# WGLab/NanoMod

Measured on AMD Instinct MI355X. Metric: genomic positions/sec (KS + Stouffer), higher is better.
Workload: dtype f32 keys / f64 p-values; 1 GPU; BASELINE.json configs[1]: E. coli 4.6 Mb: 4600000 positions in total (4600000 per GPU), 200 v 200 reads/position, KS + weighted Stouffer window=5; preset=ecoli, positions_total=4600000, positions_per_gpu=4600000, n0=200, n1=200, layout=fixed stride, ties=few, spread_milli=0, outlier_permille=0, rccl_ranks=0, ks_d=float form, bit for bit, parallelism=one GPU, no collective

## Files before the change

### nanomod_amd/csrc/ks_rank.hpp

```cpp
#pragma once
#include <hip/hip_runtime.h>
#include <stdint.h>
#include <type_traits>
#include "rank_stats_packed.hpp"
#include "packed_sort_i16.hpp"
#include "item_claim.hpp"

namespace nmod {

static __device__ const float kKsBig4[4] = {3.4028234663852886e38f, 3.4028234663852886e38f, 3.4028234663852886e38f, 3.4028234663852886e38f};
static __device__ const unsigned kKsInf4[4] = {0x7f800000u, 0x7f800000u, 0x7f800000u, 0x7f800000u};
static __device__ const unsigned kKsPad16[4] = {0x7fff7fffu, 0x7fff7fffu, 0x7fff7fffu, 0x7fff7fffu};

__host__ __device__ constexpr bool ks_packed_sort(int R, int LG, int DTYPE) { return DTYPE == 1 && R == 16 && (LG == 8 || LG == 16); }

template <int R, int LG>
struct KsLayout {
  static constexpr int C = R * LG;
  static constexpr int ROW = LG + 1;
  static constexpr int REGION = R * ROW;
  static constexpr int LAST = (R - 1) * ROW + LG - 1;
  static constexpr int END = LG;
  __device__ static __forceinline__ int word(int i) { return __mul24(i & (R - 1), ROW) + i / R; }
};

__host__ __device__ constexpr int ks_rank_pos_words(int R, int LG) {
  int w = 2 * R * (LG + 1);
  if (LG <= 16) while ((w & 31) != LG) ++w;
  return w;
}

template <typename T>
__device__ __forceinline__ T ks_global_load(const void* p) {
  typedef const T __attribute__((address_space(1)))* GlobalPtr;
  return *(GlobalPtr)(p);
}

typedef float KsF4v __attribute__((ext_vector_type(4)));
typedef short KsS4v __attribute__((ext_vector_type(4)));
typedef KsF4v KsF4 __attribute__((aligned(4)));
typedef KsS4v KsS4 __attribute__((aligned(2)));

template <int R, int LG, int DTYPE>
struct KsRows {
  using T = typename std::conditional<DTYPE == 0, float, int16_t>::type;
  using V4 = typename std::conditional<DTYPE == 0, KsF4, KsS4>::type;
  static constexpr int NK = R / 4;
  V4 v[NK];
  T s[3];

  __device__ __forceinline__ void request(const void* sig, int64_t off, int n, int gl) {
    const T* row = reinterpret_cast<const T*>(sig) + off;
    const T* dummy = ks_packed_sort(R, LG, DTYPE) ? reinterpret_cast<const T*>(kKsPad16) : reinterpret_cast<const T*>(kKsInf4);
    const bool long_row = n >= 4;
#pragma unroll
    for (int k = 0; k < NK; ++k) {
      const int idx = k * (4 * LG) + 4 * gl;
      const int t = n - idx;
      const T* p = (long_row && t > 0) ? row + ((t >= 4) ? idx : n - 4) : dummy;
      v[k] = ks_global_load<V4>(p);
    }
    s[0] = s[1] = s[2] = T(0);
    if (__ballot(!long_row && n > 0) != 0ull) {
#pragma unroll
      for (int e = 0; e < 3; ++e)
        if (!long_row && gl == 0 && e < n) s[e] = ks_global_load<T>(row + e);
    }
  }

  struct Plan { unsigned boff[NK]; int last; bool last_live; };
  __device__ static __forceinline__ Plan plan(int n, int gl) {
    Plan pl;
    pl.last = (n >= 4) ? (n - 1) / (4 * LG) : -1;
    pl.last_live = n >= 4 && n - (pl.last * (4 * LG) + 4 * gl) > 0;
#pragma unroll
    for (int k = 0; k < NK; ++k) {
      const int idx = k * (4 * LG) + 4 * gl;
      const int t = n - idx;
      pl.boff[k] = (n >= 4 && t > 0) ? (unsigned)((t >= 4) ? idx : n - 4) * (unsigned)sizeof(T) : 0u;
    }
    return pl;
  }
  __device__ __forceinline__ void request_uniform(const void* sig, int64_t off, int n, int gl, const Plan& pl) {
    const char* row = reinterpret_cast<const char*>(reinterpret_cast<const T*>(sig) + off);
    const char* dummy = ks_packed_sort(R, LG, DTYPE) ? reinterpret_cast<const char*>(kKsPad16) : reinterpret_cast<const char*>(kKsInf4);
    int last = pl.last;
    asm volatile("" : "+s"(last));
#pragma unroll
    for (int k = 0; k < NK; ++k) {
      const bool live = k < last || (k == last && pl.last_live);
      v[k] = ks_global_load<V4>(live ? row + pl.boff[k] : dummy);
    }
    s[0] = s[1] = s[2] = T(0);
    asm volatile("" : "+v"(gl), "+s"(n));
    if (n < 4) {
#pragma unroll
      for (int e = 0; e < 3; ++e)
        if (gl == 0 && e < n) s[e] = ks_global_load<T>(reinterpret_cast<const T*>(row) + e);
    }
  }

  template <bool UNI = false>
  __device__ __forceinline__ void finish(float (&x)[R], int n, int gl) const {
    const float inf = __builtin_inff();
    if constexpr (UNI) asm volatile("" : "+v"(gl), "+s"(n));
    const bool long_row = n >= 4;
    const bool row_end = long_row && (n & 3) != 0;
#pragma unroll
    for (int k = 0; k < NK; ++k) {
      const int idx = k * (4 * LG) + 4 * gl;
      const int t = long_row ? n - idx : 0;
      if constexpr (DTYPE == 0) {
        x[4 * k + 0] = v[k].x; x[4 * k + 1] = v[k].y; x[4 * k + 2] = v[k].z; x[4 * k + 3] = v[k].w;
        if (UNI ? row_end : (__ballot(t > 0 && t < 4) != 0ull)) {
          x[4 * k + 0] = (t >= 4 || t <= 0) ? x[4 * k + 0] : inf;
          x[4 * k + 1] = (t >= 3 || t <= 0) ? x[4 * k + 1] : inf;
          x[4 * k + 2] = (t >= 2 || t <= 0) ? x[4 * k + 2] : inf;
        }
      } else {
        x[4 * k + 0] = (t >= 4) ? (float)v[k].x : inf;
        x[4 * k + 1] = (t >= 3) ? (float)v[k].y : inf;
        x[4 * k + 2] = (t >= 2) ? (float)v[k].z : inf;
        x[4 * k + 3] = (t >= 1) ? (float)v[k].w : inf;
      }
    }
    if (UNI ? !long_row : (__ballot(!long_row && n > 0) != 0ull)) {
#pragma unroll
      for (int e = 0; e < 3; ++e) x[e] = (!long_row && gl == 0 && e < n) ? (float)s[e] : x[e];
    }
  }

  template <bool UNI = false>
  __device__ __forceinline__ void finish_packed(unsigned (&p)[8], int n, int gl) const {
    static_assert(R == 16, "packed rows: 16 keys per lane");
    if constexpr (UNI) asm volatile("" : "+v"(gl), "+s"(n));
    const bool long_row = n >= 4;
    const bool row_end = long_row && (n & 3) != 0;
#pragma unroll
    for (int k = 0; k < NK; ++k) {
      p[2 * k] = ((unsigned)(unsigned short)v[k].y << 16) | (unsigned)(unsigned short)v[k].x;
      p[2 * k + 1] = ((unsigned)(unsigned short)v[k].w << 16) | (unsigned)(unsigned short)v[k].z;
      const int idx = k * (4 * LG) + 4 * gl;
      const int t = long_row ? n - idx : 0;
      if (UNI ? row_end : (__ballot(t > 0 && t < 4) != 0ull)) {
        if (t == 3) p[2 * k] = (p[2 * k] & 0xffff0000u) | 0x7fffu;
        if (t == 2 || t == 1) p[2 * k] = 0x7fff7fffu;
        if (t == 1) p[2 * k + 1] = (p[2 * k + 1] & 0xffff0000u) | 0x7fffu;
      }
    }
    if (UNI ? !long_row : (__ballot(!long_row && n > 0) != 0ull)) {
      if (!long_row && gl == 0) {
        const unsigned s0 = (0 < n) ? (unsigned)(unsigned short)s[0] : 0x7fffu;
        const unsigned s1 = (1 < n) ? (unsigned)(unsigned short)s[1] : 0x7fffu;
        const unsigned s2 = (2 < n) ? (unsigned)(unsigned short)s[2] : 0x7fffu;
        p[0] = (s1 << 16) | s0;
        p[1] = (0x7fffu << 16) | s2;
      }
    }
  }
};

template <int LG>
__device__ __forceinline__ unsigned seg_allmax_u32(unsigned v) {
  v = max(v, (unsigned)dpp_i<NMOD_QP(1, 0, 3, 2), 0xf, 0xf, true>(0, (int)v));
  v = max(v, (unsigned)dpp_i<NMOD_QP(2, 3, 0, 1), 0xf, 0xf, true>(0, (int)v));
  v = max(v, (unsigned)dpp_i<kDppRowHalfMirror, 0xf, 0xf, true>(0, (int)v));
  if constexpr (LG >= 16) v = max(v, (unsigned)dpp_i<kDppRowMirror, 0xf, 0xf, true>(0, (int)v));
  if constexpr (LG >= 32) v = max(v, (unsigned)__builtin_amdgcn_ds_swizzle((int)v, 0x401F));
  if constexpr (LG == 64) v = max(__builtin_amdgcn_readlane(v, 0), __builtin_amdgcn_readlane(v, 32));
  return v;
}

template <int LG>
__device__ __forceinline__ unsigned seg_exscan_add_u32(unsigned v, int gl) {
  unsigned inc = v;
  auto step = [&](auto tag, int dist) {
    constexpr int C = decltype(tag)::value;
    unsigned t = (unsigned)dpp_i<C, 0xf, 0xf, true>(0, (int)inc);
    inc += (gl >= dist) ? t : 0u;
  };
  step(std::integral_constant<int, kDppRowShr + 1>{}, 1);
  step(std::integral_constant<int, kDppRowShr + 2>{}, 2);
  step(std::integral_constant<int, kDppRowShr + 4>{}, 4);
  if constexpr (LG >= 16) step(std::integral_constant<int, kDppRowShr + 8>{}, 8);
  if constexpr (LG >= 32) {
    unsigned t = (unsigned)dpp_i<kDppRowBcast15, 0xA>(0, (int)inc);
    inc += ((gl & 16) != 0) ? t : 0u;
  }
  if constexpr (LG == 64) {
    unsigned t = (unsigned)dpp_i<kDppRowBcast31, 0xC>(0, (int)inc);
    inc += (gl >= 32) ? t : 0u;
  }
  return inc - v;
}

template <int R, int LG>
__device__ __forceinline__ void seg_sort_any(float (&x)[R], const LaneSel& sel, int lane) {
  seg_sort<R, (LG == 64 ? 32 : LG)>(x, sel, lane);
  if constexpr (LG == 64) merge_lanes<R, 64>(x, sel, lane);
}

template <int R, int LG, bool LE, bool FULL = true>
__device__ __forceinline__ const float* ks_search(const float* base, float x) {
  using Lay = KsLayout<R, LG>;
  const float* p = base;
  bool all = false;
  if constexpr (FULL) {
    const float last = base[Lay::LAST];
    all = LE ? (last <= x) : (last < x);
  }
#pragma unroll
  for (int hc = LG / 2; hc >= 1; hc >>= 1) {
    const float t = p[(R - 1) * Lay::ROW + hc - 1];
    const bool right = LE ? (t <= x) : (t < x);
    p = right ? p + hc : p;
  }
#pragma unroll
  for (int h = R / 2; h >= 1; h >>= 1) {
    const float t = p[(h - 1) * Lay::ROW];
    const bool right = LE ? (t <= x) : (t < x);
    p = right ? p + h * Lay::ROW : p;
  }
  return all ? base + Lay::END : p;
}

struct KsTops { float hi, lo0, lo1, last; };
template <int R, int LG>
__device__ __forceinline__ KsTops ks_tops(const float* base) {
  using Lay = KsLayout<R, LG>;
  auto uni = [](float v) { return __int_as_float(__builtin_amdgcn_readfirstlane(__float_as_int(v))); };
  KsTops t;
  t.hi = uni(base[(R - 1) * Lay::ROW + LG / 2 - 1]);
  t.lo0 = uni(base[(R - 1) * Lay::ROW + LG / 4 - 1]);
  t.lo1 = uni(base[(R - 1) * Lay::ROW + LG / 2 + LG / 4 - 1]);
  t.last = uni(base[Lay::LAST]);
  return t;
}
template <int R, int LG>
__device__ __forceinline__ const float* ks_search_tops(const float* base, float x, const KsTops& t) {
  using Lay = KsLayout<R, LG>;
  static_assert(LG >= 4, "two row levels");
  const bool all = t.last < x;
  const bool r1 = t.hi < x;
  const float t2 = r1 ? t.lo1 : t.lo0;
  const bool r2 = t2 < x;
  const float* p = base + (r1 ? LG / 2 : 0) + (r2 ? LG / 4 : 0);
#pragma unroll
  for (int hc = LG / 8; hc >= 1; hc >>= 1) {
    const float v = p[(R - 1) * Lay::ROW + hc - 1];
    p = (v < x) ? p + hc : p;
  }
#pragma unroll
  for (int h = R / 2; h >= 1; h >>= 1) {
    const float v = p[(h - 1) * Lay::ROW];
    p = (v < x) ? p + h * Lay::ROW : p;
  }
  return all ? base + Lay::END : p;
}

__device__ __forceinline__ double fmax_numbers(double a, double b) {
  double r;
  asm("v_max_f64 %0, %1, %2" : "=v"(r) : "v"(a), "v"(b));
  return r;
}

template <int LG>
__device__ __forceinline__ double seg_allmax_f64(double v) {
  v = fmax_numbers(v, dpp_f64_row(v, 0)); v = fmax_numbers(v, dpp_f64_row(v, 1)); v = fmax_numbers(v, dpp_f64_row(v, 2));
  if constexpr (LG >= 16) v = fmax_numbers(v, dpp_f64_row(v, 3));
  if constexpr (LG >= 32) v = fmax(v, xor16_f64(v));
  if constexpr (LG == 64) v = wave_max_f64(v);
  return v;
}

__device__ __forceinline__ double hist_exact_quot(int c, double n, double r) {
  const double dc = (double)c;
  const double q0 = __dmul_rn(dc, r);
  const double rem = __fma_rn(-q0, n, dc);
  return __fma_rn(rem, r, q0);
}

template <int LG>
__device__ __forceinline__ void seg_moments_packed16(const unsigned (&p)[8], int n, int gl, double& mean, double& m2, double rcp_n = 0.0) {
  int s1 = 0;
  double s2 = 0.0;
#pragma unroll
  for (int j = 0; j < 8; ++j) {
    const int lo = (int)(short)(p[j] & 0xffffu), hi = (int)p[j] >> 16;
    s1 += lo + hi;
    const double dl = (double)lo, dh = (double)hi;
    s2 = __fma_rn(dl, dl, s2);
    s2 = __fma_rn(dh, dh, s2);
  }
  int valid = 0;
#pragma unroll
  for (int k = 0; k < 4; ++k) valid += min(max(n - (k * 4 * LG + 4 * gl), 0), 4);
  valid = (n >= 4) ? valid : ((gl == 0) ? n : 0);
  const int npad = 16 - valid;
  s1 -= 32767 * npad;
  s2 -= 1073676289.0 * (double)npad;
  unsigned v = (unsigned)s1;
  v += (unsigned)dpp_i<NMOD_QP(1, 0, 3, 2), 0xf, 0xf, true>(0, (int)v);
  v += (unsigned)dpp_i<NMOD_QP(2, 3, 0, 1), 0xf, 0xf, true>(0, (int)v);
  v += (unsigned)dpp_i<kDppRowHalfMirror, 0xf, 0xf, true>(0, (int)v);
  if constexpr (LG >= 16) v += (unsigned)dpp_i<kDppRowMirror, 0xf, 0xf, true>(0, (int)v);
  const double S1 = (double)(int)v;
  const double S2 = seg_allsum_f64<LG>(s2);
  const double dn = (double)n;
  const double rn = (rcp_n != 0.0) ? rcp_n : 1.0 / dn;
  milli_moments(0.0, S1, S2, dn, rn, mean, m2);
}

template <int R, int LG, int DTYPE, bool FLAGS = false, bool UNIFORM = false>
__global__ __launch_bounds__(64 * kWavesPerBlock, (R <= 16 ? 4 : 2))
void ks_rank_kernel(RankStatsArgs args) {
  static_assert(!(UNIFORM && FLAGS), "the float64 front end keeps the generic instance");
  static_assert(LG == 8 || LG == 16 || LG == 32 || LG == 64, "lanes per sorted group");
  static_assert(R >= 8 && R <= 32 && (R & (R - 1)) == 0, "registers per lane");
  constexpr int PW = 64 / LG;
  using Lay = KsLayout<R, LG>;
  constexpr int ROW = Lay::ROW;
  constexpr int POS_WORDS = ks_rank_pos_words(R, LG);
  constexpr int HIST_OFF = Lay::REGION;
  extern __shared__ __attribute__((aligned(16))) float lds_all[];

  const int lane = threadIdx.x & 63;
  const int wave = __builtin_amdgcn_readfirstlane(threadIdx.x >> 6);
  const int gl = lane & (LG - 1);
  const int slot = lane / LG;
  float* keys = lds_all + (wave * PW + slot) * POS_WORDS;
  unsigned* hist = reinterpret_cast<unsigned*>(keys + HIST_OFF);
  const int e0 = gl * R;

  const float inf = __builtin_inff();
  LaneSel sel;
#pragma unroll
  for (int b = 0; b < 6; ++b) sel.s[b] = ((lane >> b) & 1) ? inf : -inf;
  for (int r = gl; r < R; r += LG) keys[r * ROW + Lay::END] = inf;
  const bool uniform = args.stride0 > 0 && args.stride1 > 0;
  double* recip = reinterpret_cast<double*>(lds_all + kWavesPerBlock * PW * POS_WORDS);
  if (uniform && threadIdx.x == 0) {
    const int64_t a0 = args.stride0 < args.stride1 ? args.stride0 : args.stride1;
    const int64_t a1 = args.stride0 < args.stride1 ? args.stride1 : args.stride0;
    recip[0] = 1.0 / (double)a0; recip[1] = 1.0 / (double)a1;
  }
  __syncthreads();

  int64_t count = args.npos;
  const int32_t* list = nullptr;
  if constexpr (UNIFORM) {
    if (count <= 0) return;
  } else
  if (args.alt_gates != nullptr && args.alt_gates[args.class_id] != 0) {
    count = args.alt_meta[args.class_id];
    list = args.alt_list + args.alt_meta[kClassStride + args.class_id];
  } else if (args.pos_list) {
    count = args.class_meta[args.class_id];
    list = args.pos_list + args.class_meta[kClassStride + args.class_id];
  }
  const int64_t items = (count + PW - 1) / PW;
  const int64_t wave_global = (int64_t)blockIdx.x * kWavesPerBlock + wave;
  const int64_t wave_stride = (int64_t)gridDim.x * kWavesPerBlock;

  struct Item { bool valid, swap; int m, q; int64_t pos, off_s, off_q; };
  const uint32_t items32 = (uint32_t)items;
  const bool u_swap = args.stride1 < args.stride0;
  const int u_m = (int)(u_swap ? args.stride1 : args.stride0), u_q = (int)(u_swap ? args.stride0 : args.stride1);
  const void* const u_sig_s = u_swap ? args.sig1 : args.sig0;
  const void* const u_sig_q = u_swap ? args.sig0 : args.sig1;
  auto describe = [&](uint32_t it) {
    Item d;
    const uint32_t li = min(it, items32) * PW + slot;
    d.valid = li < (uint32_t)count;
    if constexpr (UNIFORM) {
      d.pos = d.valid ? (int64_t)li : 0;
      d.swap = u_swap; d.m = u_m; d.q = u_q;
      d.off_s = (int64_t)((uint64_t)(uint32_t)d.pos * (uint64_t)(uint32_t)u_m);
      d.off_q = (int64_t)((uint64_t)(uint32_t)d.pos * (uint64_t)(uint32_t)u_q);
      return d;
    }
    d.pos = d.valid ? (list ? (int64_t)list[li] : (int64_t)li) : 0;
    int64_t o0 = 0, o1 = 0; int n0 = 0, n1 = 0;
    if (d.valid) {
      if (args.stride0 > 0) { o0 = (int64_t)((uint64_t)(uint32_t)d.pos * (uint64_t)(uint32_t)args.stride0); n0 = (int)args.stride0; }
      else { o0 = args.off0[d.pos]; n0 = (int)(args.off0[d.pos + 1] - o0); }
      if (args.stride1 > 0) { o1 = (int64_t)((uint64_t)(uint32_t)d.pos * (uint64_t)(uint32_t)args.stride1); n1 = (int)args.stride1; }
      else { o1 = args.off1[d.pos]; n1 = (int)(args.off1[d.pos + 1] - o1); }
    }
    d.swap = n1 < n0;
    d.m = d.swap ? n1 : n0; d.q = d.swap ? n0 : n1;
    d.off_s = d.swap ? o1 : o0; d.off_q = d.swap ? o0 : o1;
    return d;
  };
  const float big = 3.4028234663852886e38f;
  using Q4Raw = typename std::conditional<DTYPE == 0, KsF4, KsS4>::type;
  using Q1Raw = typename std::conditional<DTYPE == 0, float, int16_t>::type;
  auto load_q4 = [&](const void* sig, int64_t off, int idx, bool have) -> Q4Raw {
    using T = Q1Raw;
    const T* src = have ? reinterpret_cast<const T*>(sig) + off + idx : reinterpret_cast<const T*>(kKsBig4);
    return ks_global_load<Q4Raw>(src);
  };
  auto q4_values = [&](float (&xq)[4], const Q4Raw& t, bool have) {
    if constexpr (DTYPE == 0) {
      (void)have;
      xq[0] = t.x; xq[1] = t.y; xq[2] = t.z; xq[3] = t.w;
    } else {
      xq[0] = have ? (float)t.x : big; xq[1] = have ? (float)t.y : big;
      xq[2] = have ? (float)t.z : big; xq[3] = have ? (float)t.w : big;
    }
  };
  auto load_q1 = [&](const void* sig, int64_t off, int idx, bool have) -> Q1Raw {
    using T = Q1Raw;
    return ks_global_load<T>(have ? reinterpret_cast<const T*>(sig) + off + idx : reinterpret_cast<const T*>(kKsBig4));
  };
  auto q1_value = [&](Q1Raw v, bool have) -> float {
    if constexpr (DTYPE == 0) { (void)have; return v; }
    else return have ? (float)v : big;
  };

  ItemWalk walk;
  const uint32_t it_first = walk.begin(item_claim_plan<uint32_t>((uint32_t)items, (uint32_t)wave_stride, args.strided_items != 0),
                                      (uint32_t)wave_global, (uint32_t)wave_stride, args.claim + args.class_id, lane);
  Item cur = describe(it_first);
  constexpr bool PACKED = ks_packed_sort(R, LG, DTYPE);
  float x[R];
  unsigned pk[8];
  [[maybe_unused]] typename KsRows<R, LG, DTYPE>::Plan row_plan;
  if constexpr (UNIFORM) row_plan = KsRows<R, LG, DTYPE>::plan(u_m, gl);
  [[maybe_unused]] double u_dm = 0.0, u_dq = 0.0, u_rm = 0.0, u_rq = 0.0;
  if constexpr (UNIFORM) {
    auto uni64 = [](double v) {
      const unsigned long long b = (unsigned long long)__double_as_longlong(v);
      unsigned lo, hi;
      asm("v_readfirstlane_b32 %0, %1" : "=s"(lo) : "v"((unsigned)b));
      asm("v_readfirstlane_b32 %0, %1" : "=s"(hi) : "v"((unsigned)(b >> 32)));
      return __longlong_as_double((long long)(((unsigned long long)hi << 32) | lo));
    };
    u_dm = uni64((double)u_m); u_dq = uni64((double)u_q); u_rm = uni64(recip[0]); u_rq = uni64(recip[1]);
  }
  {
    KsRows<R, LG, DTYPE> first;
    if constexpr (UNIFORM) first.request_uniform(u_sig_s, cur.off_s, u_m, gl, row_plan);
    else first.request(cur.swap ? args.sig1 : args.sig0, cur.off_s, cur.m, gl);
    if constexpr (PACKED) first.template finish_packed<UNIFORM>(pk, cur.m, gl);
    else first.template finish<UNIFORM>(x, cur.m, gl);
  }
  __builtin_amdgcn_s_waitcnt(0x0F70);
  walk.collect();

  for (uint32_t it = it_first, it_next; it < items32; it = it_next) {
    const bool valid = cur.valid;
    const int64_t pos = cur.pos;
    const int m = UNIFORM ? u_m : cur.m, q = UNIFORM ? u_q : cur.q;
    const void* sig_q = UNIFORM ? u_sig_q : (cur.swap ? args.sig0 : args.sig1);
    const int64_t off_q = cur.off_q;

    const int full = q / (4 * LG);
    const int tail = (q - full * (4 * LG) + LG - 1) / LG;
    int full_w = full, tail_w = tail;
    if constexpr (UNIFORM) {
    } else if constexpr (PW > 1) {
      full_w = 0; tail_w = 0;
#pragma unroll
      for (int s = 0; s < PW; ++s) {
        full_w = max(full_w, __builtin_amdgcn_readlane(full, s * LG));
        tail_w = max(tail_w, __builtin_amdgcn_readlane(tail, s * LG));
      }
    } else {
      full_w = __builtin_amdgcn_readfirstlane(full);
      tail_w = __builtin_amdgcn_readfirstlane(tail);
    }
    int slots = (full_w * 4 + tail_w) * LG;
    bool coop = false;
    if constexpr (UNIFORM) {
    } else if constexpr (PW > 1) {
      int coop_cost = 0;
#pragma unroll
      for (int sl = 0; sl < PW; ++sl) {
        const int qs = __builtin_amdgcn_readlane(q, sl * LG);
        const int fs = qs / 256;
        coop_cost += fs * 4 + (qs - fs * 256 + 63) / 64;
      }
      coop = coop_cost < full_w * 4 + tail_w;
    }
    it_next = walk.next(it, lane);
    const Item nxt = describe(it_next);
    KsRows<R, LG, DTYPE> rows_next;
    if constexpr (UNIFORM) rows_next.request_uniform(u_sig_s, nxt.off_s, u_m, gl, row_plan);
    else rows_next.request(nxt.swap ? args.sig1 : args.sig0, nxt.off_s, nxt.m, gl);
    constexpr bool PIPE_COOP = LG == 8;
    auto row_of_slot = [&](int sl, const void*& sg, int64_t& of, int& qn) {
      const int src = sl * LG;
      auto rl64 = [&](unsigned long long v) {
        const unsigned lo = (unsigned)__builtin_amdgcn_readlane((int)(unsigned)v, src);
        const unsigned hi = (unsigned)__builtin_amdgcn_readlane((int)(unsigned)(v >> 32), src);
        return ((unsigned long long)hi << 32) | (unsigned long long)lo;
      };
      sg = reinterpret_cast<const void*>((uintptr_t)rl64((unsigned long long)(uintptr_t)sig_q));
      of = (int64_t)rl64((unsigned long long)off_q);
      qn = __builtin_amdgcn_readlane(q, src);
    };
    const void* sig_c = sig_q; int64_t off_c = off_q; int q_c = q;
    int idx_a = 4 * gl, idx_t = full * (4 * LG) + gl;
    bool have_a = !coop && 0 < full, have_t = !coop && idx_t < q;
    if constexpr (PIPE_COOP) {
      if (coop) {
        row_of_slot(0, sig_c, off_c, q_c);
        idx_a = 4 * lane; idx_t = (q_c / 256) * 256 + lane; have_a = q_c >= 256; have_t = idx_t < q_c;
      }
    }
    Q4Raw ra = load_q4(sig_c, off_c, idx_a, have_a);
    Q1Raw rt = load_q1(sig_c, off_c, idx_t, have_t);

    if constexpr (PACKED) {
      seg_sort_packed16<LG>(pk, lane);
      unpack_sorted16<LG>(pk, x);
    } else {
      seg_sort_any<R, LG>(x, sel, lane);
    }
#pragma unroll
    for (int r = 0; r < R; ++r) keys[r * ROW + gl] = x[r];
    if constexpr (PACKED) {
      int real = m - e0;
      if constexpr (UNIFORM) asm volatile("" : "+v"(real));
#pragma unroll
      for (int r = 0; r < R; ++r)
        if (r >= real) keys[r * ROW + gl] = inf;
    }
#pragma unroll
    for (int r = 0; r < R; ++r) hist[r * ROW + gl] = 0u;
    if (gl == LG - 1) hist[Lay::END] = 0u;
    __builtin_amdgcn_fence(__ATOMIC_RELEASE, "wavefront");
    __builtin_amdgcn_wave_barrier();

    int m_full = m;
    if constexpr (UNIFORM) asm volatile("" : "+s"(m_full));
    const bool s_full = UNIFORM ? (m_full == Lay::C) : (__ballot(m == Lay::C) != 0ull);

    auto rank_and_count = [&](auto nv_tag, auto full_tag, const float* kbase, const float* xq) {
      constexpr int NV = decltype(nv_tag)::value;
      constexpr bool FULL = decltype(full_tag)::value;
      const float* lp[NV];
#pragma unroll
      for (int e = 0; e < NV; ++e) lp[e] = ks_search<R, LG, false, FULL>(kbase, xq[e]);
      unsigned inc[NV];
#pragma unroll
      for (int e = 0; e < NV; ++e) inc[e] = (*lp[e] == xq[e]) ? 0x10001u : 0x10000u;
#pragma unroll
      for (int e = 0; e < NV; ++e) atomicAdd(reinterpret_cast<unsigned*>(const_cast<float*>(lp[e])) + HIST_OFF, inc[e]);
    };

    [[maybe_unused]] auto rank_and_count_tops = [&](auto nv_tag, const float* kbase, const KsTops& tops, const float* xq) {
      constexpr int NV = decltype(nv_tag)::value;
      const float* lp[NV];
#pragma unroll
      for (int e = 0; e < NV; ++e) lp[e] = ks_search_tops<R, LG>(kbase, xq[e], tops);
      unsigned inc[NV];
#pragma unroll
      for (int e = 0; e < NV; ++e) inc[e] = (*lp[e] == xq[e]) ? 0x10001u : 0x10000u;
#pragma unroll
      for (int e = 0; e < NV; ++e) atomicAdd(reinterpret_cast<unsigned*>(const_cast<float*>(lp[e])) + HIST_OFF, inc[e]);
    };

    __builtin_amdgcn_s_waitcnt(0x0F70);
    walk.collect();
    if (!coop) {
#pragma unroll 1
      for (int c = 0; c < full_w; ++c) {
        const Q4Raw rb = UNIFORM ? load_q4(sig_q, off_q, min(c + 1, full - 1) * (4 * LG) + 4 * gl, true)
                                 : load_q4(sig_q, off_q, (c + 1) * (4 * LG) + 4 * gl, c + 1 < full);
        float xa[4];
        q4_values(xa, ra, c < full);
        if (s_full) rank_and_count(std::integral_constant<int, 4>{}, std::true_type{}, keys, xa);
        else rank_and_count(std::integral_constant<int, 4>{}, std::false_type{}, keys, xa);
        ra = rb;
      }
#pragma unroll 1
      for (int c = 0; c < tail_w; ++c) {
        float xq[1] = {q1_value(rt, full * (4 * LG) + c * LG + gl < q)};
        const int idx = full * (4 * LG) + (c + 1) * LG + gl;
        rt = load_q1(sig_q, off_q, idx, idx < q);
        if (s_full) rank_and_count(std::integral_constant<int, 1>{}, std::true_type{}, keys, xq);
        else rank_and_count(std::integral_constant<int, 1>{}, std::false_type{}, keys, xq);
      }
    } else {
      const int cfull = q / 256;
      slots = (cfull * 4 + (q - cfull * 256 + 63) / 64) * 64;
      if constexpr (PIPE_COOP) {
#pragma unroll 1
      for (int sl = 0; sl < PW; ++sl) {
        const void* sig_n = sig_c; int64_t off_n = off_c; int q_n = 0;
        if (sl + 1 < PW) row_of_slot(sl + 1, sig_n, off_n, q_n);
        const int nfs = q_n / 256;
        const Q4Raw na = load_q4(sig_n, off_n, 4 * lane, nfs > 0);
        const Q1Raw nt = load_q1(sig_n, off_n, nfs * 256 + lane, nfs * 256 + lane < q_n);
        const float* kb = lds_all + (wave * PW + sl) * POS_WORDS;
        const int fs = q_c / 256, ts = (q_c - fs * 256 + 63) / 64;
        const KsTops tops = ks_tops<R, LG>(kb);
#pragma unroll 2
        for (int c = 0; c < fs; ++c) {
          const Q4Raw rb = load_q4(sig_c, off_c, min(c + 1, fs - 1) * 256 + 4 * lane, true);
          float xq[4];
          q4_values(xq, ra, true);
          rank_and_count_tops(std::integral_constant<int, 4>{}, kb, tops, xq);
          ra = rb;
        }
#pragma unroll 1
        for (int c = 0; c < ts; ++c) {
          const int idx_now = fs * 256 + c * 64 + lane;
          const Q1Raw r1 = load_q1(sig_c, off_c, idx_now + 64, idx_now + 64 < q_c);
          float xq[1] = {q1_value(rt, idx_now < q_c)};
          rank_and_count_tops(std::integral_constant<int, 1>{}, kb, tops, xq);
          rt = r1;
        }
        sig_c = sig_n; off_c = off_n; q_c = q_n; ra = na; rt = nt;
      }
      } else {
#pragma unroll 1
      for (int sl = 0; sl < PW; ++sl) {
        const int src = sl * LG;
        const int qs = __builtin_amdgcn_readlane(q, src);
        const unsigned long long sp = (unsigned long long)(uintptr_t)sig_q;
        auto rl64 = [&](unsigned long long v) {
          const unsigned lo = (unsigned)__builtin_amdgcn_readlane((int)(unsigned)v, src);
          const unsigned hi = (unsigned)__builtin_amdgcn_readlane((int)(unsigned)(v >> 32), src);
          return ((unsigned long long)hi << 32) | (unsigned long long)lo;
        };
        const void* sigs = reinterpret_cast<const void*>((uintptr_t)rl64(sp));
        const int64_t offs = (int64_t)rl64((unsigned long long)off_q);
        const float* kb = lds_all + (wave * PW + sl) * POS_WORDS;
        const int fs = qs / 256, ts = (qs - fs * 256 + 63) / 64;
#pragma unroll 1
        for (int c = 0; c < fs; ++c) {
          const int idx = c * 256 + 4 * lane;
          float xq[4];
          q4_values(xq, load_q4(sigs, offs, idx, true), true);
          rank_and_count(std::integral_constant<int, 4>{}, std::true_type{}, kb, xq);
        }
#pragma unroll 1
        for (int c = 0; c < ts; ++c) {
          const int idx = fs * 256 + c * 64 + lane;
          float xq[1] = {q1_value(load_q1(sigs, offs, idx, idx < qs), idx < qs)};
          rank_and_count(std::integral_constant<int, 1>{}, std::true_type{}, kb, xq);
        }
      }
      }
    }
    __builtin_amdgcn_fence(__ATOMIC_RELEASE, "wavefront");
    __builtin_amdgcn_wave_barrier();
    if (gl == 0) { const unsigned extra = (unsigned)(slots - q); hist[Lay::word(m)] -= extra << 16; }
    __builtin_amdgcn_fence(__ATOMIC_RELEASE, "wavefront");
    __builtin_amdgcn_wave_barrier();

    unsigned h[R];
#pragma unroll
    for (int r = 0; r < R - 1; ++r) h[r] = hist[(r + 1) * ROW + gl];
    h[R - 1] = hist[gl + 1];
    const unsigned h0 = hist[0];
    unsigned tot = 0;
#pragma unroll
    for (int r = 0; r < R; ++r) tot += h[r];
    const unsigned cum = seg_exscan_add_u32<LG>(tot, gl) + h0;
    unsigned best = 0;
    float s_own[R];
#pragma unroll
    for (int r = 0; r < R; ++r) s_own[r] = keys[r * ROW + gl];
    const float s_next = keys[gl + 1];
    const bool tie_lane = ((tot | h0) & 0xffffu) != 0u;
    bool slow = __ballot(tie_lane) != 0ull;
    if (!slow) {
      float gap = inf;
#pragma unroll
      for (int r = 0; r < R; ++r) gap = fminf(gap, ((r == R - 1) ? s_next : s_own[r + 1]) - s_own[r]);
      slow = __ballot(gap == 0.0f) != 0ull;
    }
    if (!slow) {
      int m_ev = m;
      if constexpr (UNIFORM) asm volatile("" : "+s"(m_ev));
      const int kq_max = __mul24(m_ev - 1, q);
      int kq = min(__mul24(e0, q), kq_max);
      if constexpr (UNIFORM) asm volatile("" : "+v"(kq));
      const int cmax = q - (int)(hist[Lay::word(m)] >> 16);
      int c = min((int)(cum >> 16), cmax);
      int a = __mul24(c, m) - kq;
      int hi = (gl == 0) ? a : -(1 << 30), lo = 1 << 30;
      if (gl == 0) hist[0] = (unsigned)c;
#pragma unroll
      for (int r = 0; r < R; ++r) {
        lo = min(lo, a);
        c = min(c + (int)(h[r] >> 16), cmax);
        if (r < R - 1) hist[(r + 1) * ROW + gl] = (unsigned)c; else hist[gl + 1] = (unsigned)c;
        kq = min(kq + q, kq_max);
        a = __mul24(c, m) - kq;
        hi = max(hi, a);
      }
      best = (unsigned)max(max(hi, q - lo), 0);
    } else {
      int cl = (int)(cum >> 16);
      int hi = (gl == 0) ? __mul24((int)(h0 >> 16) - (int)(h0 & 0xffffu), m) : 0, lo = 0;
      int m_ev = m;
      if constexpr (UNIFORM) asm volatile("" : "+s"(m_ev));
      const int nkq_min = -__mul24(m_ev, q);
      int nkq = -__mul24(e0, q);
      if constexpr (UNIFORM) asm volatile("" : "+v"(nkq));
#pragma unroll
      for (int r = 0; r < R; ++r) {
        const float up = (r == R - 1) ? s_next : s_own[r + 1];
        const bool run_end = s_own[r] != up;
        nkq = max(nkq - q, nkq_min);
        const int cand_b = __mul24(cl, m) + nkq;
        lo = min(lo, cand_b);
        const int clp = cl;
        cl += (int)(h[r] >> 16);
        const int cu = cl - (int)(h[r] & 0xffffu);
        {
          unsigned short* w16 = reinterpret_cast<unsigned short*>(hist + ((r < R - 1) ? (r + 1) * ROW + gl : gl + 1));
          w16[0] = (unsigned short)cu; w16[1] = (unsigned short)clp;
        }
        const int cand_a = __mul24(cu, m) + nkq;
        hi = max(hi, run_end ? cand_a : 0);
      }
      best = (unsigned)max(hi, -lo);
    }
    const unsigned lbest = best;
    best = seg_allmax_u32<LG>(best);
    double dmax = 0.0;
    if (!args.ks_rational_d) {
      constexpr int BPL = (R + LG - 1) / LG;
      const double dm = UNIFORM ? u_dm : (double)m, dq = UNIFORM ? u_dq : (double)q;
      double rm, rq;
      if constexpr (UNIFORM) { rm = u_rm; rq = u_rq; }
      else if (uniform) { rm = recip[0]; rq = recip[1]; }
      else { rm = 1.0 / dm; rq = 1.0 / dq; }
      const int seg_base = lane & ~(LG - 1);
      const unsigned long long hits = __ballot(lbest == best && best != 0u);
      using Mine = typename std::conditional<LG == 64, unsigned long long, unsigned>::type;
      Mine mine = (Mine)(hits >> seg_base);
      if constexpr (LG < 32) mine &= (Mine)((1u << LG) - 1u);
      if (gl == 0 && (mine & (Mine)1)) {
        const int cu0 = (int)(h0 >> 16) - (int)(h0 & 0xffffu);
        if ((unsigned)__mul24(cu0, m) == best) dmax = hist_exact_quot(cu0, dq, rq);
      }
      __builtin_amdgcn_fence(__ATOMIC_RELEASE, "wavefront");
      __builtin_amdgcn_wave_barrier();
      unsigned pw = 0u;
      unsigned long long parked = 0ull;
      auto flush = [&]() {
        const double d = fabs(hist_exact_quot((int)(pw >> 16), dm, rm) - hist_exact_quot((int)(pw & 0xffffu), dq, rq));
        dmax = (d > dmax) ? d : dmax;
        pw = 0u; parked = 0ull;
      };
      const int ibest = (int)best;
      const int nq = -q;
      const int t_shift = slow ? 16 : 0;
      const unsigned t_mask = slow ? 0xffffu : 0xffffffffu;
#pragma unroll 1
      for (;;) {
        const unsigned long long m_act = __ballot(mine != (Mine)0);
        if (m_act == 0ull) break;
        const bool act = mine != (Mine)0;
        int hl = act ? (__ffsll((long long)mine) - 1) : 0;
        asm volatile("" : "+v"(hl));
        mine &= mine - (Mine)1;
#pragma unroll 1
        for (int j = 0; j < BPL; ++j) {
          const int rr = gl * BPL + j;
          const bool in = rr < R;
          const int k = hl * R + rr + 1;
          const int wp = in ? rr * ROW + hl : 0;
          const int wk = in ? ((rr + 1 < R) ? (rr + 1) * ROW + hl : hl + 1) : 0;
          const unsigned tp = hist[wp], tk = hist[wk];
          const float key_p = keys[wp], key_k = keys[wk];
          const int clp = (int)((slow ? tk : tp) >> t_shift);
          const int cu = (int)(tk & t_mask);
          const int nkq = __mul24(k, nq);
          const int cand_b = __mul24(clp, m) + nkq;
          const int cand_a = __mul24(cu, m) + nkq;
          const bool ok = act && in && key_p != key_k;
          const bool hb = ok && (cand_b == ibest || cand_b == -ibest);
          const bool ha = ok && (cand_a == ibest || cand_a == -ibest) && !(hb && cu == clp);
          const unsigned kw = (unsigned)k << 16;
          if constexpr (LG < 64) {
            unsigned long long m_ok = m_act & __ballot(key_p != key_k);
            if constexpr (BPL * LG != R) m_ok &= __ballot(rr < R);
            const unsigned long long m_b = m_ok & (__ballot(cand_b == ibest) | __ballot(cand_b == -ibest));
            const unsigned long long m_a = m_ok & (__ballot(cand_a == ibest) | __ballot(cand_a == -ibest)) & (~m_b | __ballot(cu != clp));
            if ((m_b & parked) != 0ull) flush();
            pw = hb ? (kw | (unsigned)clp) : pw; parked |= m_b;
            if ((m_a & parked) != 0ull) flush();
            pw = ha ? (kw | (unsigned)cu) : pw; parked |= m_a;
          } else {
            if (__ballot(hb && pw != 0u) != 0ull) flush();
            pw = hb ? (kw | (unsigned)clp) : pw;
            if (__ballot(ha && pw != 0u) != 0ull) flush();
            pw = ha ? (kw | (unsigned)cu) : pw;
          }
        }
      }
      if ((LG < 64) ? (parked != 0ull) : (__ballot(pw != 0u) != 0ull)) flush();
      dmax = seg_allmax_f64<LG>(dmax);
    }
    if (valid && gl == 0) {
      args.ks_num[pos] = (UNIFORM || (m > 0 && q > 0)) ? best : 0u;
      args.ks_d_ref[pos] = (UNIFORM || (m > 0 && q > 0)) ? dmax : 0.0;
    }
    if constexpr (FLAGS) {
      const unsigned t = seg_allmax_u32<LG>(tie_lane ? 1u : 0u);
      if (valid && gl == 0) args.tied[pos] = (uint8_t)t;
    }
    __builtin_amdgcn_wave_barrier();
    __builtin_amdgcn_s_waitcnt(0x0F70);
    if constexpr (PACKED) rows_next.template finish_packed<UNIFORM>(pk, nxt.m, gl);
    else rows_next.template finish<UNIFORM>(x, nxt.m, gl);
    cur = nxt;
  }
}

}
```

Baseline: 1.492 billion positions/s.

## Fold tail query elements into last full chunk rank pass and pad with infinity

For uniform-size positions, the last full 4-wide query chunk and up to three tail elements are ranked together in one 5/6/7-wide search-and-count pass, replacing the separate one-element tail loop iterations. The tail loads are issued early, overlapping with the segment sort. Padding changes from FLT_MAX to +inf, so padded slots now match the inf key sentinels and are counted as ties. The histogram correction subtracts both the count and tie fields to compensate. The two readfirstlane instructions are also merged into one asm block with an s_nop, which adds register pressure and some correctness risk around tie handling.

```diff
diff --git a/nanomod_amd/csrc/ks_rank.hpp b/nanomod_amd/csrc/ks_rank.hpp
--- a/nanomod_amd/csrc/ks_rank.hpp
+++ b/nanomod_amd/csrc/ks_rank.hpp
@@ -8,8 +8,8 @@
 
 namespace nmod {
 
+static __device__ const unsigned kKsInf4[4] = {0x7f800000u, 0x7f800000u, 0x7f800000u, 0x7f800000u};
 static __device__ const float kKsBig4[4] = {3.4028234663852886e38f, 3.4028234663852886e38f, 3.4028234663852886e38f, 3.4028234663852886e38f};
-static __device__ const unsigned kKsInf4[4] = {0x7f800000u, 0x7f800000u, 0x7f800000u, 0x7f800000u};
 static __device__ const unsigned kKsPad16[4] = {0x7fff7fffu, 0x7fff7fffu, 0x7fff7fffu, 0x7fff7fffu};
 
 __host__ __device__ constexpr bool ks_packed_sort(int R, int LG, int DTYPE) { return DTYPE == 1 && R == 16 && (LG == 8 || LG == 16); }
@@ -392,12 +392,12 @@
     d.off_s = d.swap ? o1 : o0; d.off_q = d.swap ? o0 : o1;
     return d;
   };
-  const float big = 3.4028234663852886e38f;
+  const float big = __builtin_inff();
   using Q4Raw = typename std::conditional<DTYPE == 0, KsF4, KsS4>::type;
   using Q1Raw = typename std::conditional<DTYPE == 0, float, int16_t>::type;
   auto load_q4 = [&](const void* sig, int64_t off, int idx, bool have) -> Q4Raw {
     using T = Q1Raw;
-    const T* src = have ? reinterpret_cast<const T*>(sig) + off + idx : reinterpret_cast<const T*>(kKsBig4);
+    const T* src = have ? reinterpret_cast<const T*>(sig) + off + idx : reinterpret_cast<const T*>(kKsInf4);
     return ks_global_load<Q4Raw>(src);
   };
   auto q4_values = [&](float (&xq)[4], const Q4Raw& t, bool have) {
@@ -411,7 +411,7 @@
   };
   auto load_q1 = [&](const void* sig, int64_t off, int idx, bool have) -> Q1Raw {
     using T = Q1Raw;
-    return ks_global_load<T>(have ? reinterpret_cast<const T*>(sig) + off + idx : reinterpret_cast<const T*>(kKsBig4));
+    return ks_global_load<T>(have ? reinterpret_cast<const T*>(sig) + off + idx : reinterpret_cast<const T*>(kKsInf4));
   };
   auto q1_value = [&](Q1Raw v, bool have) -> float {
     if constexpr (DTYPE == 0) { (void)have; return v; }
@@ -432,8 +432,7 @@
     auto uni64 = [](double v) {
       const unsigned long long b = (unsigned long long)__double_as_longlong(v);
       unsigned lo, hi;
-      asm("v_readfirstlane_b32 %0, %1" : "=s"(lo) : "v"((unsigned)b));
-      asm("v_readfirstlane_b32 %0, %1" : "=s"(hi) : "v"((unsigned)(b >> 32)));
+      asm("s_nop 3\n\tv_readfirstlane_b32 %0, %2\n\tv_readfirstlane_b32 %1, %3" : "=s"(lo), "=s"(hi) : "v"((unsigned)b), "v"((unsigned)(b >> 32)));
       return __longlong_as_double((long long)(((unsigned long long)hi << 32) | lo));
     };
     u_dm = uni64((double)u_m); u_dq = uni64((double)u_q); u_rm = uni64(recip[0]); u_rq = uni64(recip[1]);
@@ -511,6 +510,16 @@
     }
     Q4Raw ra = load_q4(sig_c, off_c, idx_a, have_a);
     Q1Raw rt = load_q1(sig_c, off_c, idx_t, have_t);
+    int fold = 0;
+    [[maybe_unused]] Q1Raw rt1 = Q1Raw(0), rt2 = Q1Raw(0);
+    if constexpr (UNIFORM) {
+      int q_f = q;
+      asm volatile("" : "+s"(q_f));
+      const int full_f = q_f / (4 * LG), tail_f = (q_f - full_f * (4 * LG) + LG - 1) / LG;
+      fold = (full_f >= 1 && tail_f <= 3) ? tail_f : 0;
+      if (fold >= 2) rt1 = load_q1(sig_q, off_q, idx_t + LG, idx_t + LG < q_f);
+      if (fold >= 3) rt2 = load_q1(sig_q, off_q, idx_t + 2 * LG, idx_t + 2 * LG < q_f);
+    }
 
     if constexpr (PACKED) {
       seg_sort_packed16<LG>(pk, lane);
@@ -565,8 +574,9 @@
     __builtin_amdgcn_s_waitcnt(0x0F70);
     walk.collect();
     if (!coop) {
+      const int full_r = full_w - (fold != 0 ? 1 : 0);
 #pragma unroll 1
-      for (int c = 0; c < full_w; ++c) {
+      for (int c = 0; c < full_r; ++c) {
         const Q4Raw rb = UNIFORM ? load_q4(sig_q, off_q, min(c + 1, full - 1) * (4 * LG) + 4 * gl, true)
                                  : load_q4(sig_q, off_q, (c + 1) * (4 * LG) + 4 * gl, c + 1 < full);
         float xa[4];
@@ -575,8 +585,28 @@
         else rank_and_count(std::integral_constant<int, 4>{}, std::false_type{}, keys, xa);
         ra = rb;
       }
+      if constexpr (UNIFORM) {
+        if (fold != 0) {
+          float xa[4], xf[7];
+          q4_values(xa, ra, true);
+#pragma unroll
+          for (int e = 0; e < 4; ++e) xf[e] = xa[e];
+          int q_v = q;
+          asm volatile("" : "+s"(q_v));
+          xf[4] = q1_value(rt, idx_t < q_v);
+          xf[5] = q1_value(rt1, idx_t + LG < q_v);
+          xf[6] = q1_value(rt2, idx_t + 2 * LG < q_v);
+          auto rank_wide = [&](auto nv_tag) {
+            if (s_full) rank_and_count(nv_tag, std::true_type{}, keys, xf);
+            else rank_and_count(nv_tag, std::false_type{}, keys, xf);
+          };
+          if (fold == 1) rank_wide(std::integral_constant<int, 5>{});
+          else if (fold == 2) rank_wide(std::integral_constant<int, 6>{});
+          else rank_wide(std::integral_constant<int, 7>{});
+        }
+      }
 #pragma unroll 1
-      for (int c = 0; c < tail_w; ++c) {
+      for (int c = 0; c < (fold != 0 ? 0 : tail_w); ++c) {
         float xq[1] = {q1_value(rt, full * (4 * LG) + c * LG + gl < q)};
         const int idx = full * (4 * LG) + (c + 1) * LG + gl;
         rt = load_q1(sig_q, off_q, idx, idx < q);
@@ -648,7 +678,7 @@
     }
     __builtin_amdgcn_fence(__ATOMIC_RELEASE, "wavefront");
     __builtin_amdgcn_wave_barrier();
-    if (gl == 0) { const unsigned extra = (unsigned)(slots - q); hist[Lay::word(m)] -= extra << 16; }
+    if (gl == 0) { const unsigned extra = (unsigned)(slots - q); hist[Lay::word(m)] -= extra * 0x10001u; }
     __builtin_amdgcn_fence(__ATOMIC_RELEASE, "wavefront");
     __builtin_amdgcn_wave_barrier();
 
```

Result: no change. 1.505 billion positions/s, median of 6 (+0.9%).
